# bonjour-l/esa-pose-estimation

Hardware: AMD Instinct MI355X
Metric: HRNet-W32 256x256 crops/sec (heatmaps + fused argmax/refine keypoints) (higher is better)
Workload: dtype bf16x6 (fp32-grade: every f32 operand split exactly into 3 bf16 terms, 6 bf16 MFMAs per product, f32 accumulate; f32 NHWC activations; f32 VALU stem conv1 / output layer) — heat-maps closer to fp64 than the fp32 CPU reference; 1 GPU; seg_hrnet2 HRNet-W32 256x256, batch 32/GPU, 11 keypoints, fp32 NCHW in -> heatmaps -> keypoints (BASELINE configs[1]); global_batch=32, per_gpu_batch=32, parallelism=dp1, hip_graph=True

## Files before the change

esa-pose-estimation_amd/csrc/conv_x6.hip:

```cpp
#include <algorithm>
#include <atomic>
#include <cstdio>
#include <type_traits>

#include "conv_cfg.h"
#include "devstate.h"
#include "kernels.h"
#include "sb.h"

#ifdef X6_TRACE
__device__ unsigned long long g_x6_trace[64 * 32 * 8];
extern "C" int esa_debug_x6_trace(void* dst) { return (int)hipMemcpyFromSymbol(dst, HIP_SYMBOL(g_x6_trace), sizeof(g_x6_trace)); }
__device__ unsigned long long g_x6_wg[1024 * 8];
extern "C" int esa_debug_x6_wg(void* dst) { return (int)hipMemcpyFromSymbol(dst, HIP_SYMBOL(g_x6_wg), sizeof(g_x6_wg)); }
#endif

#ifndef X6_ABL
#define X6_ABL 0
#endif
#ifndef X6_KG_SKEW
#define X6_KG_SKEW 1
#endif
#ifndef X6_W2BUF
#define X6_W2BUF 1
// ... 175 lines not shown
    auto advance = [&](const X6Pos& a) {
        X6Pos q = a;
        if (q.c + 1 < nchunks) {
            ++q.c;
        } else {
            q.c = 0;
            q.item += G;
            q.ok = a.ok && q.item < geo.nitems;
            if (q.ok) decode(q);
        }
        return q;
    };

    float* const w1s = reinterpret_cast<float*>(smem + C::LDS);
    constexpr int RW = C::IW + 2, RH = C::IH + 2, RAWN = RW * RH, RIT = STEM ? (RAWN + C::NT - 1) / C::NT : 1;
    float* const rawt = w1s + 2 * 4 * 10 * 8;
    if (STEM) {
        for (int i = tid; i < 2 * 4 * 10 * 8; i += C::NT) w1s[i] = stem.w1[i];
    }
    const int sg = tid & 3, q0 = tid >> 2;
    int qyx[XITER];
#pragma unroll
    for (int it = 0; it < XITER; ++it) {
        const int q = q0 + it * QSTEP;
        const int qy = q / C::IW, qx = q - qy * C::IW;
        qyx[it] = q < C::NPIX ? (qy << 8 | qx) : -1;
    }
    int roff[STEM ? XITER : 1];
    if constexpr (STEM) {
#pragma unroll
        for (int it = 0; it < XITER; ++it) roff[it] = qyx[it] >= 0 ? (qyx[it] >> 8) * RW + (qyx[it] & 255) : 0;
    }
    constexpr bool DEEP = !STEM && NBUF == 2 && (S == 2 || KS == 1) && X6_DEEP;
    constexpr int XH = (KS == 1 || DEEP || NBUF == 1) ? XITER : (XITER + 1) / 2;
    u32x4 xr[STEM ? 1 : XH][2];
// ... 66 lines not shown
                const int i = tid + k * C::NT;
                const int ry = i / RW, rx_ = i - ry * RW;
                const int yy = gy0 + ry, xx = gx0 + rx_;
                const bool in = i < RAWN && (unsigned)yy < (unsigned)p.H && (unsigned)xx < (unsigned)p.W;
                rawreg[k] = __builtin_bit_cast(float, __builtin_amdgcn_raw_buffer_load_b32(rx, in ? (yy * p.W + xx) * 4 : (int)X6_OOB, 0, 0));
            }
        }
    };
    auto raw_commit = [&](int rb) __attribute__((always_inline)) {
        if constexpr (STEM) {
#pragma unroll
            for (int k = 0; k < RIT; ++k)
                if (RAWN % C::NT == 0 || k + 1 < RIT || tid + k * C::NT < RAWN) rawt[rb * RAWN + tid + k * C::NT] = rawreg[k];
        }
    };
    auto stage_stem = [&](int buf, const X6Pos& q, int rb) __attribute__((always_inline)) {
        if constexpr (STEM) {
            const float* wt = w1s + (q.c * 4 + sg) * 80;
            const float* rt = rawt + rb * RAWN;
            const int gy0 = q.oy0 * S - C::PAD, gx0 = q.ox0 * S - C::PAD;
            constexpr int UG = XITER <= 3 ? 3 : 2;
            x6_static_for<0, (XITER + UG - 1) / UG>([&](auto g_c) __attribute__((always_inline)) {
                constexpr int u0 = decltype(g_c)::value * UG, un = XITER - u0 < UG ? XITER - u0 : UG;
                f32x4 a0[un], a1[un];
                {
                    const f32x4 b0 = *reinterpret_cast<const f32x4*>(wt + 72), b1 = *reinterpret_cast<const f32x4*>(wt + 76);
#pragma unroll
                    for (int u = 0; u < un; ++u) { a0[u] = b0; a1[u] = b1; }
                }
                x6_static_for<0, 9>([&](auto t_c) __attribute__((always_inline)) {
                    constexpr int t = decltype(t_c)::value;
                    const f32x4 w0 = *reinterpret_cast<const f32x4*>(wt + t * 8), w1v = *reinterpret_cast<const f32x4*>(wt + t * 8 + 4);
                    x6_static_for<0, un>([&](auto u_c) __attribute__((always_inline)) {
                        constexpr int u = decltype(u_c)::value;
                        const float v = rt[roff[u0 + u] + (t / 3) * RW + t % 3];
                        a0[u] = __builtin_elementwise_fma(f32x4{v, v, v, v}, w0, a0[u]);
                        a1[u] = __builtin_elementwise_fma(f32x4{v, v, v, v}, w1v, a1[u]);
                    });
                });
                x6_static_for<0, un>([&](auto u_c) __attribute__((always_inline)) {
                    constexpr int u = decltype(u_c)::value, it = u0 + u;
                    const int gy = gy0 + (qyx[it] >> 8), gx = gx0 + (qyx[it] & 255);
                    const uint32_t m = (qyx[it] >= 0 && (unsigned)gy < (unsigned)p.H && (unsigned)gx < (unsigned)p.W) ? 0xffffffffu : 0u;
                    u32x4 src[2];
#pragma unroll
                    for (int k = 0; k < 4; ++k) {
                        src[0][k] = __float_as_uint(relu1(a0[u][k])) & m;
                        src[1][k] = __float_as_uint(relu1(a1[u][k])) & m;
                    }
                    emit_unit(buf, it, src);
                });
                __builtin_amdgcn_sched_barrier(0);
// ... 694 lines not shown
    if (nblk <= 0 || nblk > 0x7fffffffLL) return (int)hipErrorInvalidValue;
    const int ntile16 = p.Coutp >> 4;
    long long want = (4LL * device_cus() + nblk - 1) / nblk;
    if (want > ntile16 / 4) want = ntile16 / 4;
    const int slices = want < 1 ? 1 : (int)want;
    const int per = (ntile16 + slices - 1) / slices;
    auto kern = conv1x1_x6_kernel<NCH, PG>;
    if (const int e_ = ensure_dyn_lds(reinterpret_cast<const void*>(kern), lds + per * 64)) return e_;
    hipLaunchKernelGGL(kern, dim3((unsigned)nblk, (unsigned)((ntile16 + per - 1) / per)), dim3(NTHREADS), lds + per * 64, stream, p, ntiles, tiles_per_row, per);
    return (int)hipGetLastError();
}

bool stem_fused_x6_supported(int cin, int cmid, int coutp) { return X6_MODE == 2 && cin == 1 && cmid == 64 && coutp % 64 == 0; }

void pack_stem_w1_x6(const float* w, const float* b, float* dst) {
    for (int c = 0; c < 2; ++c)
        for (int sg = 0; sg < 4; ++sg)
            for (int j = 0; j < 8; ++j) {
                const int ch = c * 32 + x6_chan_of_k(sg, j);
                float* o = dst + (c * 4 + sg) * 80;
                for (int t = 0; t < 9; ++t) o[t * 8 + j] = w[ch * 9 + t];
                o[72 + j] = b[ch];
            }
}

int launch_stem_fused_x6(const StemFusedParams& sp, hipStream_t stream) {
    if (!stem_fused_x6_supported(sp.cin, sp.Cmid, sp.Coutp)) return (int)hipErrorInvalidValue;
    using C = X6Cfg<3, 2, 4, X6_STEM_NR, 4, X6_STEM_NBUF>;
    ConvParams p{};
    p.x = nullptr; p.y = sp.y; p.res = nullptr; p.w = sp.w2; p.bias = sp.bias2;
    p.N = sp.N; p.H = sp.H; p.W = sp.W; p.OH = sp.OH; p.OW = sp.OW; p.Cinp = sp.Cmid; p.Coutp = sp.Coutp; p.relu = 1; p.fmt = FMT_F32;
    if (sp.OH != (sp.H + 1) / 2 || sp.OW != (sp.W + 1) / 2 || (long long)sp.H * sp.W * 4 >= 0x7fffffffLL ||
        (long long)sp.OH * sp.OW * sp.Coutp * 4 >= 0x7fffffffLL)
        return (int)hipErrorInvalidValue;
    X6Geo geo;
    geo.tiles_x = (p.OW + TW - 1) / TW;
    geo.tiles_y = (p.OH + C::TH - 1) / C::TH;
    geo.ctiles = p.Coutp / 64;
    const long long nitems = (long long)p.N * geo.tiles_y * geo.tiles_x * geo.ctiles;
    if (nitems <= 0 || nitems > 0x7fffffffLL) return (int)hipErrorInvalidValue;
    geo.nitems = (int)nitems;
    geo.m_ct = x6_magic(geo.ctiles);
    geo.m_tx = x6_magic(geo.tiles_x);
    geo.m_ty = x6_magic(geo.tiles_y);
    const int slots = 2 * device_cus();
    int grid = (int)(nitems < slots ? nitems : slots);
    if (grid > geo.ctiles) grid -= grid % geo.ctiles;
    constexpr int LDS = C::LDS + 2 * 4 * 10 * 8 * 4 + 2 * (C::IW + 2) * (C::IH + 2) * 4;
    if (const int e_ = ensure_dyn_lds(reinterpret_cast<const void*>(stem_x6_kernel), LDS)) return e_;
    X6StemSrc src{sp.x, sp.w1};
    hipLaunchKernelGGL(stem_x6_kernel, dim3((unsigned)grid), dim3(NTHREADS), LDS, stream, p, geo, src);
    return (int)hipGetLastError();
}

bool conv1x1_x6_supported(const ConvParams& p) {
    const int n = p.Cinp / 32;
    return p.fmt == FMT_F32 && !p.res && !p.out_f32 && p.nheads <= 1 && (p.Cinp % 32) == 0 && (p.Coutp % 16) == 0 && p.H == p.OH &&
           p.W == p.OW && (n == 1 || n == 2 || n == 3 || n == 4 || n == 6 || n == 8) && p.Coutp >= X6_C1_MINCOUT;
}
int launch_conv1x1_x6(const ConvParams& p, hipStream_t stream) {
    if (!conv1x1_x6_supported(p)) return (int)hipErrorInvalidValue;
    switch (p.Cinp / 32) {
        case 1: return launch_c1_x6_t<1, 2>(p, stream);
// ... 75 lines not shown
```

esa-pose-estimation_amd/csrc/head.hip:

```cpp
#include "devstate.h"
#include "gaussfit.h"
#include "kernels.h"
#include "refine.h"
#include "sb.h"

namespace esa {
namespace {

constexpr int FTW = 32;
constexpr int FIW = FTW + 2;
constexpr int FROW = FIW + 1;

struct LerpT {
    int i0, i1;
    float l0, l1;
};
__device__ __forceinline__ LerpT lerp_ac_true(int dst, int in, int out) {
    const float scale = out > 1 ? (float)(in - 1) / (float)(out - 1) : 0.f;
    const float src = scale * (float)dst;
    LerpT r;
    r.i0 = min((int)src, in - 1);
    r.i1 = r.i0 + (r.i0 < in - 1 ? 1 : 0);
    r.l1 = src - (float)r.i0;
    r.l0 = 1.f - r.l1;
// ... 35 lines not shown
        ld(r0 + lx.i1, v01);
        ld(r1 + lx.i0, v10);
        ld(r1 + lx.i1, v11);
#pragma unroll
        for (int i = 0; i < 8; ++i)
            v[i] = ly.l0 * (lx.l0 * v00[i] + lx.l1 * v01[i]) + ly.l1 * (lx.l0 * v10[i] + lx.l1 * v11[i]);
    }
}
__device__ __forceinline__ float final_stage_raw(const FinalParams& p, int n, int ci, int gy, int gx) {
    float v = 0.f;
    if (gy >= 0 && gy < p.H && gx >= 0 && gx < p.W)
        v = p.x0[(((size_t)n * p.cin + ci) * p.H + gy) * p.W + gx];
    return v;
}

template <int RPT>
__device__ __forceinline__ void final_tile_max(const FinalParams& p, const float* red, int tiles_x, int tiles_y) {
    constexpr int NP = FTW * 8 * RPT;
    const int lane = threadIdx.x & 63;
    const int ntiles = tiles_x * tiles_y, tile = (int)(blockIdx.x % (unsigned)ntiles), n = (int)(blockIdx.x / (unsigned)ntiles);
    const int oy0 = tile / tiles_x * (8 * RPT), ox0 = tile % tiles_x * FTW;
    for (int k = threadIdx.x >> 6; k < p.K; k += 4) {
        float bv = -INFINITY;
        int bi = 0x7fffffff;
#pragma unroll
        for (int j = 0; j < NP / 64; ++j) {
            const int q = lane + 64 * j, oy = oy0 + q / FTW, ox = ox0 + q % FTW;
            if (oy < p.H && ox < p.W) argmax_take(red[k * NP + q], oy * p.W + ox, bv, bi);
        }
#pragma unroll
// ... 6 lines not shown
    }
}

template <int KT, int RPT, bool KP>
__global__ __launch_bounds__(256) void final_kernel(FinalParams p, int tiles_x, int tiles_y) {
    constexpr int FTH = 8 * RPT, FIH = FTH + 2;
    extern __shared__ __attribute__((aligned(16))) char smem[];
    float* tile = reinterpret_cast<float*>(smem);
    const int CT = p.K + p.cin;
    int b = blockIdx.x;
    const int tx = b % tiles_x; b /= tiles_x;
    const int ty = b % tiles_y;
    const int n = b / tiles_y;
    const int oy0 = ty * FTH, ox0 = tx * FTW;

    constexpr int G = (KT + 7) >> 3;
    const float sc_y = final_scale(p.h, p.H), sc_x = final_scale(p.wd, p.W);
    for (int u = threadIdx.x; u < FIH * FIW * G; u += 256) {
        const int c8 = u % G;
        const int q = u / G;
        const int py = q / FIW, px = q - py * FIW;
        const int gy = oy0 - 1 + py, gx = ox0 - 1 + px;
        float v[8];
        final_stage8(p, n, gy, gx, c8, sc_y, sc_x, v);
#pragma unroll
        for (int i = 0; i < 8; ++i) {
            const int c = c8 * 8 + i;
            if (c < p.K) tile[(c * FIH + py) * FROW + px] = v[i];
        }
    }
    for (int u = threadIdx.x; u < FIH * FIW * p.cin; u += 256) {
        const int px = u % FIW;
        const int r = u / FIW;
        const int py = r % FIH, ci = r / FIH;
        tile[((p.K + ci) * FIH + py) * FROW + px] = final_stage_raw(p, n, ci, oy0 - 1 + py, ox0 - 1 + px);
    }
    __syncthreads();

    const int lx = threadIdx.x & (FTW - 1), lyy = (threadIdx.x / FTW) * RPT;
    if constexpr (RPT == 2) {
        f32x2 acc[KT];
#pragma unroll
        for (int k = 0; k < KT; ++k) acc[k] = f32x2{p.bias[k], p.bias[k]};
        for (int c = 0; c < CT; ++c) {
            const float* tp = tile + (c * FIH + lyy) * FROW + lx;
            const float* wp = p.w + (size_t)c * 9 * KT;
            float r[4][3];
#pragma unroll
            for (int i = 0; i < 4; ++i)
#pragma unroll
                for (int j = 0; j < 3; ++j) r[i][j] = tp[i * FROW + j];
// ... 66 lines not shown
    const int tiles_x = (p.W + FTW - 1) / FTW, tiles_y = (p.H + FTH - 1) / FTH;
    const long long nblk = (long long)p.N * tiles_x * tiles_y;
    if (nblk <= 0 || nblk > 0x7fffffffLL) return (int)hipErrorInvalidValue;
    const size_t lds = (size_t)(p.K + p.cin) * FIH * FROW * sizeof(float);
    auto kern = final_kernel<KT, RPT, KP>;
    if (const int e_ = ensure_dyn_lds(reinterpret_cast<const void*>(kern), 64 * 1024)) return e_;
    if (lds > 64 * 1024) return (int)hipErrorInvalidValue;
    hipLaunchKernelGGL(kern, dim3((unsigned)nblk), dim3(256), lds, stream, p, tiles_x, tiles_y);
    return (int)hipGetLastError();
}
inline int final_rpt(int K, int cin, int KT) { return (size_t)(K + cin) * 18 * FROW * sizeof(float) <= 64 * 1024 && KT <= 16 ? 2 : 1; }
template <int KT, bool KP = false>
int launch_final_t(const FinalParams& p, hipStream_t stream) {
    if (final_rpt(p.K, p.cin, KT) == 2) return launch_final_rt<KT, 2, KP>(p, stream);
    return launch_final_rt<KT, 1, KP>(p, stream);
}

constexpr int FKP_MAXC = 40;
__global__ __launch_bounds__(64) void final_kp_finish_kernel(FinalParams p, int kt, int ntiles, float* kp, int* idx_out) {
    __shared__ float sv[81][FKP_MAXC];
    __shared__ float spt[9];
    const int plane = blockIdx.x, n = plane / p.K, k = plane - n * p.K;
    float bv;
    int bi;
    reduce_tile_maxima(p.part + (size_t)plane * ntiles, ntiles, bv, bi);
    const int b0 = bi == 0x7fffffff ? 0 : bi, px = b0 % p.W, py = b0 / p.W;
    const int npt = 1 < px && px < p.W - 2 && 1 < py && py < p.H - 2 ? 9 : 1;
    const int G = (p.K + 7) >> 3, U = G + p.cin, CT = p.K + p.cin;
    const float sc_y = final_scale(p.h, p.H), sc_x = final_scale(p.wd, p.W);
    for (int u = threadIdx.x; u < npt * 9 * U; u += 64) {
// ... 492 lines not shown
            for (int l = 0; l < 64; ++l)
                for (int j = 0; j < 8; ++j) {
                    const int co = m * 16 + (l & 15), G = c * 4 + (l >> 4);
                    float v = 0.f;
                    if (G < 9 * cg_n) {
                        const int tap = G / cg_n, ch = (G % cg_n) * 8 + j;
                        if (co < K && ch < ct) v = w[((size_t)co * ct + ch) * 9 + tap];
                    }
                    const uint16_t hi = fb16(v), lo = fb16(v - fb16f(hi));
                    const size_t base = (((size_t)m * nch + c) * 2) * 512;
                    d[base + l * 8 + j] = hi;
                    d[base + 512 + l * 8 + j] = lo;
                }
}

int final_kp_tiles(int K, int cin, int H, int W) {
    const int kt = final_kt(K);
    if (kt < 0 || H <= 0 || W <= 0) return 0;
    return ((W + FTW - 1) / FTW) * ((H + 8 * final_rpt(K, cin, kt) - 1) / (8 * final_rpt(K, cin, kt)));
}

int launch_final_kp(const FinalParams& p, float* kp, int* idx_out, hipStream_t stream) {
    const int ntiles = final_kp_tiles(p.K, p.cin, p.H, p.W), kt = final_kt(p.K);
    const long long planes = (long long)p.N * p.K;
    if (!p.part || !kp || ntiles <= 0 || p.K + p.cin > FKP_MAXC || planes > 0x7fffffffLL || (long long)p.H * p.W > 0x7fffffffLL)
        return (int)hipErrorInvalidValue;
    int rc = (int)hipErrorInvalidValue;
    switch (kt) {
        case 11: rc = launch_final_t<11, true>(p, stream); break;
        case 16: rc = launch_final_t<16, true>(p, stream); break;
// ... 68 lines not shown
                case 31: return launch_final_mfma_t<3, 1, true>(p, stream);
                case 32: return launch_final_mfma_t<3, 2, true>(p, stream);
                case 42: return launch_final_mfma_t<4, 2, true>(p, stream);
                case 52: return launch_final_mfma_t<5, 2, true>(p, stream);
            }
        }
        switch (cg * 10 + m) {
            case 21: return launch_final_mfma_t<2, 1>(p, stream);
            case 31: return launch_final_mfma_t<3, 1>(p, stream);
            case 32: return launch_final_mfma_t<3, 2>(p, stream);
            case 42: return launch_final_mfma_t<4, 2>(p, stream);
            case 52: return launch_final_mfma_t<5, 2>(p, stream);
        }
    }
    if (p.fmt == FMT_HF) return (int)hipErrorInvalidValue;
    switch (final_kt(p.K)) {
        case 11: return launch_final_t<11>(p, stream);
        case 16: return launch_final_t<16>(p, stream);
        case 32: return launch_final_t<32>(p, stream);
    }
    return (int)hipErrorInvalidValue;
}

}
```

esa-pose-estimation_amd/csrc/kernels.h:

```cpp
#pragma once
#include <hip/hip_runtime.h>
#include <stdint.h>

namespace esa {

enum { FMT_SB = 0, FMT_BF = 1, FMT_F32 = 2, FMT_HF = 3 };
inline bool fmt_half(int fmt) { return fmt == FMT_BF || fmt == FMT_HF; }

int set_error(const char* fmt, ...);

struct ConvParams {
    const char* x;
    char* y;
    const char* res;
    const uint4* w;
    const float* bias;
    int N, H, W, OH, OW;
    int Cinp, Coutp;
    int relu;
    int out_f32;
    int fmt;
    int nheads;
    int x6_reload;
    char* yh[3];
// ... 58 lines not shown
    const float* bias2;
    int N, H, W;
};
int launch_bblock32(const BlockParams& p, hipStream_t stream);

struct StemFusedParams {
    const float* x;
    char* y;
    const float* w1;
    const float* bias1;
    const uint4* w2;
    const float* bias2;
    int N, H, W, OH, OW, cin, Cmid, Coutp;
};
int launch_stem_fused(const StemFusedParams& p, hipStream_t stream);
bool stem_fused_x6_supported(int cin, int cmid, int coutp);
void pack_stem_w1_x6(const float* w, const float* b, float* dst);
int launch_stem_fused_x6(const StemFusedParams& p, hipStream_t stream);

struct FuseParams {
    const char* x[4];
    int h[4], w[4];
    int nterms;
    char* y;
    int N, H, W, Cp;
    int relu;
    int fmt;
};
int launch_fuse(const FuseParams& p, hipStream_t stream);

struct FinalParams {
    const char* h3;
    const float* x0;
    float* out;
    const float* w;
    const float* bias;
    const uint4* wpk;
    int N, H, W, h, wd;
    int K, cin, Cp;
    int fmt;
    float2* part;
};
int launch_final(const FinalParams& p, hipStream_t stream);
int final_kp_tiles(int K, int cin, int H, int W);
int launch_final_kp(const FinalParams& p, float* kp, int* idx_out, hipStream_t stream);
int launch_final_gf(const FinalParams& p, float* kp, int* idx_out, double* fit, int* status, double* hess, hipStream_t stream);
int launch_final_gf_cov(const FinalParams& p, float* kp, int* idx_out, double* fit, int* status, double* hess, double* cov,
                        double* info, double cov_floor, hipStream_t stream);
int final2_valu_tiles(int H, int W);
int launch_final2_kp(const FinalParams& p, float* bmax, float* kp, int* idx_out, hipStream_t stream, double* hess = nullptr);
int final_part_tiles(int K, int cin, int H, int W);
__device__ __forceinline__ void argmax_take(float v, int i, float& bv, int& bi) {
    const bool vn = v != v, bn = bv != bv;
    if (v > bv || (vn && !bn) || ((v == bv || (vn && bn)) && i < bi)) { bv = v; bi = i; }
}
bool final_mfma_supported(int K, int cin);
size_t final_mfma_bytes(int K, int cin);
void pack_final_mfma(const float* w, int K, int cin, void* dst);

struct HeadParams {
    const char* x0;
    const char* t[3];
    char* y;
    const uint4* w0;
    const uint4* w3;
    const float* bias0;
    const float* bias3;
    int N, H, W;
    int th[3], tw[3];
    int C0p, Ctp, C3p, K;
    bool valu;
    bool hf;
};
// ... 194 lines not shown
```

esa-pose-estimation_amd/csrc/op_abi.hip:

```cpp
#include <algorithm>
#include <cstdint>
#include <cstdio>
#include <cstring>
#include <vector>

#include "../../include/esahrnet.h"
#include "host_util.h"
#include "kernels.h"

using esa::DevScope;
using esa::Format;
using esa::set_error;

static const float* f32(const void* p) { return static_cast<const float*>(p); }
static float* f32(void* p) { return static_cast<float*>(p); }
static bool aligned(const void* p, uintptr_t a) { return (reinterpret_cast<uintptr_t>(p) & (a - 1)) == 0; }

static bool conv_form_ok(int k, int stride) { return (k == 1 && stride == 1) || (k == 3 && (stride == 1 || stride == 2)); }
static bool op_conv_dims_ok(int n, int cin, int cout, int h, int w, int k, int stride) {
    if (n <= 0 || cin <= 0 || cout <= 0 || h <= 0 || w <= 0 || !conv_form_ok(k, stride)) return false;
    return (long long)n * h * w * (long long)((std::max(cin, cout) + 63) & ~63) * 4 <= 0x7fffffffLL;
}
static esa::ConvParams op_conv_shape(const Format& f, int n, int cin, int cout, int h, int w, int stride, int relu, const void* res) {
    esa::ConvParams p{};
// ... 305 lines not shown

int esahrnet_op_stem2(const void* x_dev, int n, int cin, int height, int width, const float* w1, const float* b1, int cmid,
                      const float* w2, const float* b2, int cout, int precision, void* y_dev, esahrnet_stream stream_) {
    const char* who = "op_stem2";
    if (!x_dev || !w1 || !b1 || !w2 || !b2 || !y_dev) return set_error("%s: null argument", who);
    if (precision != 0 && precision != 2) return set_error("%s: precision %d (0: stem_fused, 2: stem_x6_kernel)", who, precision);
    const Format f(precision);
    if (cin < 1 || cin > 4) return set_error("%s: cin=%d (1 .. 4)", who, cin);
    if (cmid <= 0 || (cmid & 31)) return set_error("%s: cmid=%d (a positive multiple of 32)", who, cmid);
    if (!op_conv_dims_ok(n, cmid, cout, height, width, 3, 2)) return set_error("%s: n=%d cmid=%d cout=%d %dx%d unsupported", who, n, cmid, cout, height, width);
    const int coutp = f.pad(cout), oh = (height + 1) / 2, ow = (width + 1) / 2;
    if (f.x6 && !esa::stem_fused_x6_supported(cin, cmid, coutp)) return set_error("%s: stem_x6_kernel does not serve cin=%d cmid=%d cout=%d", who, cin, cmid, cout);
    std::vector<float> w1p, b1p(b1, b1 + cmid), b2p(coutp, 0.f);
    std::copy(b2, b2 + cout, b2p.begin());
    if (f.x6) {
        w1p.assign(2 * 4 * 10 * 8, 0.f);
        esa::pack_stem_w1_x6(w1, b1, w1p.data());
    } else {
        w1p = esa::pack_stem_w(w1, cmid, cin, cmid);
    }
    DevScope m(who, static_cast<hipStream_t>(stream_));
    esa::StemFusedParams p{};
    p.x = f32(x_dev);
    p.N = n; p.H = height; p.W = width; p.OH = oh; p.OW = ow; p.cin = cin; p.Cmid = cmid; p.Coutp = coutp;
    if (m.upload(w1p, &p.w1) || m.upload(b1p, &p.bias1) || m.upload(f.pack(w2, cout, cmid, 3, coutp, cmid), &p.w2) || m.upload(b2p, &p.bias2)) return 1;
    if (m.alloc(&p.y, (size_t)n * oh * ow * coutp * 4)) return 1;
    int rc = f.x6 ? esa::launch_stem_fused_x6(p, m.stream()) : esa::launch_stem_fused(p, m.stream());
    if (!rc) rc = esa::launch_fmt_to_nchw(f.fmt, p.y, n, coutp, oh, ow, coutp, f32(y_dev), m.stream());
    return m.finish(rc);
}

// ... 69 lines not shown
```

esa-pose-estimation_amd/csrc/plan.hip:

```cpp
#include <hip/hip_runtime.h>

#include <algorithm>
#include <cmath>
#include <cstdarg>
#include <cstdio>
#include <cstdlib>
#include <cstring>
#include <map>
#include <string>
#include <vector>

#include "../../include/esahrnet.h"
#include "devstate.h"
#include "host_util.h"
#include "kernels.h"

namespace esa {
int final_kt(int K);
extern const int kFrontendMaxRows;
int check_boxes_args(const char* who, int m, int frame_h, int frame_w, int scale, int rule);
int check_crops_args(const char* who, int nframes, int pixel_format, float stdv);
int check_cov_args(const char* who, const void* cov_dev, const void* info_dev, double cov_floor);
int check_corr_args(const char* who, int m, int k, int mode);
}
// ... 107 lines not shown
};

enum StemForm { STEM_SEPARATE, STEM_FUSED, STEM_FUSED_X6 };
enum HeadForm { HEAD_UNFUSED, HEAD_SB, HEAD_BF, HEAD_X6 };

struct PlanOptions {
    bool unfused, head_v1, final_valu, no_multihead, no_jobs, no_bblock, no_cbam_jobs, cbam_unfused, stem_pool_separate,
         head3_direct, head3_cout32, bf_unfused_head, bf_head_valu, x6_unfused_head, x6_unfused_stem, x6_reload_weights, tap_all;
    int nlanes;
    int fmt;
    StemForm stem;
    bool fused_block;
    HeadForm head;
    bool head2;
    bool final_mfma;
};

PlanOptions plan_options(const esahrnet_cfg& g, const esa::Format& format) {
    const auto on = esa::env_on;
    PlanOptions o;
    o.unfused = on("ESAHRNET_UNFUSED"); o.head_v1 = on("ESAHRNET_HEAD_V1"); o.final_valu = on("ESAHRNET_FINAL_VALU");
    o.no_multihead = on("ESAHRNET_NO_MULTIHEAD"); o.no_jobs = on("ESAHRNET_NO_JOBS"); o.no_bblock = on("ESAHRNET_NO_BBLOCK");
    o.no_cbam_jobs = on("ESAHRNET_NO_CBAM_JOBS"); o.cbam_unfused = on("ESAHRNET_CBAM_UNFUSED");
    o.stem_pool_separate = on("ESAHRNET_STEM_POOL_SEPARATE"); o.head3_direct = on("ESAHRNET_HEAD3_DIRECT");
    o.head3_cout32 = on("ESAHRNET_HEAD3_COUT32"); o.bf_unfused_head = on("ESAHRNET_BF_UNFUSED_HEAD");
    o.bf_head_valu = on("ESAHRNET_BF_HEAD_VALU"); o.x6_unfused_head = on("ESAHRNET_X6_UNFUSED_HEAD");
    o.x6_unfused_stem = on("ESAHRNET_X6_UNFUSED_STEM"); o.tap_all = on("ESAHRNET_TAP_ALL");
    o.x6_reload_weights = on("ESAHRNET_X6_RELOAD_WEIGHTS");
    const char* streams = getenv("ESAHRNET_STREAMS");
    o.nlanes = streams && atoi(streams) > 1 ? 4 : 1;
// ... 1 lines not shown
    const bool sb = o.fmt == esa::FMT_SB, v0 = g.variant == 0;
    const bool x6_stem = esa::stem_fused_x6_supported(g.cin, pad32(g.stem_width), pad32(g.stem_width)) && g.stem_width == 64;
    o.stem = sb && (!v0 || !o.unfused) ? STEM_FUSED
           : o.fmt == esa::FMT_F32 && x6_stem && !o.x6_unfused_stem ? STEM_FUSED_X6 : STEM_SEPARATE;
    o.fused_block = sb && v0 && !o.unfused && !o.no_bblock;
    int nb4 = 0;
    while (nb4 < ESAHRNET_MAX_BRANCHES && g.blocks[3][nb4] > 0) ++nb4;
    const int c0 = pad32(g.widths[0]);
    o.head = !v0 || nb4 != 4 ? HEAD_UNFUSED
           : sb ? (!o.unfused && (c0 == 32 || c0 == 64) ? HEAD_SB : HEAD_UNFUSED)
           : esa::fmt_half(o.fmt) ? (!o.bf_unfused_head && (pad64(g.widths[0]) == 64 || pad64(g.widths[0]) == 128) ? HEAD_BF : HEAD_UNFUSED)
           : !o.x6_unfused_head && (c0 == 32 || c0 == 64) ? HEAD_X6 : HEAD_UNFUSED;
    o.head2 = !o.head_v1 && (o.head != HEAD_SB || ((pad32(g.widths[1]) == 64 || pad32(g.widths[1]) == 96) &&
                                                   esa::head_t_supported(pad32(g.widths[2])) && esa::head_t_supported(pad32(g.widths[3]))));
    o.final_mfma = v0 && o.fmt != esa::FMT_F32 && !o.final_valu && esa::final_mfma_supported(g.num_keypoints, g.cin);
    return o;
}

}

int esa::set_error(const char* fmt, ...) {
    va_list ap;
    va_start(ap, fmt);
    vsnprintf(g_err, sizeof g_err, fmt, ap);
    va_end(ap);
    return 1;
}

bool esa::conv_group_mergeable(int fmt, const esa::ConvParams* ps, int n, int k, int stride) {
    if (fmt == esa::FMT_F32) return esa::conv_x6_jobs_supported(ps, n, k, stride);
// ... 12 lines not shown
                  fmt == esa::FMT_HF ? "fp16" : esa::fmt_half(fmt) ? "true" : "false");
}

struct esahrnet_ctx {
    esahrnet_cfg cfg;
    int device;
    std::vector<ConvSpec> specs;
    std::map<std::string, int> spec_by_name;
    std::vector<DevConv> dconvs;
    std::vector<AuxSpec> aux;
    float *stemraw_w = nullptr, *stemraw_b = nullptr;
    std::vector<Tensor> tensors;
    std::vector<Op> ops;
    int spec_stem = -1, spec_final = -1;
    float *stem_w = nullptr, *stem_b = nullptr, *final_w = nullptr, *final_b = nullptr;
    void* final_wpk = nullptr;
    int spec_l0 = -1, spec_l3 = -1, head_c0 = 0;
    void *head_w0 = nullptr, *head_w3 = nullptr;
    float *head_b0 = nullptr, *head_b3 = nullptr;
    bool committed = false;
    bool keep = false;
    PlanOptions opt;
    esa::Format format;
    bool h16() const { return format.half; }
    bool hf() const { return format.hf; }
    bool x6() const { return format.x6; }
    int padc(int ch) const { return format.pad(ch); }
    int eb() const { return format.eb; }
    size_t wbytes(int coutp, int cinp, int k) const { return format.wbytes(coutp, cinp, k); }
    std::vector<char> pack(const float* w, int cout, int cin, int k, int coutp, int cinp) const { return format.pack(w, cout, cin, k, coutp, cinp); }
// ... 997 lines not shown
                if (allocated[ti] && last_of(t) == (int)oi) release(t.off, bytes_of(t));
            }
        high = std::max(high, top);
    }
    sp.bytes = high;
    c.sp = sp;
    return 0;
}

void free_weights(esahrnet_ctx& c) {
    for (DevConv& d : c.dconvs) {
        if (d.w) (void)hipFree(d.w);
        if (d.bias) (void)hipFree(d.bias);
        d.w = nullptr; d.bias = nullptr;
    }
    for (float** p : {&c.stem_w, &c.stem_b, &c.final_w, &c.final_b, &c.head_b0, &c.head_b3})
        if (*p) { (void)hipFree(*p); *p = nullptr; }
    for (void** p : {&c.head_w0, &c.head_w3, &c.final_wpk})
        if (*p) { (void)hipFree(*p); *p = nullptr; }
    for (AuxSpec& a : c.aux) if (a.dev) { (void)hipFree(a.dev); a.dev = nullptr; }
    for (Multi& m : c.multis) {
        if (m.w) (void)hipFree(m.w);
        if (m.bias) (void)hipFree(m.bias);
        m.w = nullptr; m.bias = nullptr;
    }
    for (float** p : {&c.stemraw_w, &c.stemraw_b}) if (*p) { (void)hipFree(*p); *p = nullptr; }
    for (std::vector<hipEvent_t>* v : {&c.wave_entry, &c.wave_end, &c.op_event}) {
        for (hipEvent_t& e : *v) if (e) { (void)hipEventDestroy(e); e = nullptr; }
        v->clear();
    }
    for (int i = 0; i < 3; ++i) {
// ... 259 lines not shown
        size_t wo = 0, bo = 0;
        for (int k = 0; k < m.n; ++k) {
            const DevConv& d = h->dconvs[h->ops[m.op[k]].dconv];
            const size_t wb = esa::packed_weight_bytes(d.coutp, d.cinp, 3);
            HIP_OK(hipMemcpy(static_cast<char*>(m.w) + wo, d.w, wb, hipMemcpyDeviceToDevice));
            HIP_OK(hipMemcpy(m.bias + bo, d.bias, (size_t)d.coutp * sizeof(float), hipMemcpyDeviceToDevice));
            wo += wb; bo += d.coutp;
        }
    }
    {
        const ConvSpec& s = h->specs[h->spec_stem];
        const int coutp = h->padc(s.cout);
        std::vector<float> w = pack_stem_w(s.w.data(), s.cout, s.cin, coutp), b(coutp, 0.f);
        std::copy(s.b.begin(), s.b.begin() + s.cout, b.begin());
        if (h->opt.stem == STEM_FUSED_X6) {
            std::vector<float> wx(2 * 4 * 10 * 8, 0.f);
            esa::pack_stem_w1_x6(s.w.data(), s.b.data(), wx.data());
            w = wx;
        }
        if (upload(w, reinterpret_cast<void**>(&h->stem_w)) || upload(b, reinterpret_cast<void**>(&h->stem_b))) return 1;
    }
    if (h->cfg.variant == 0) {
        const ConvSpec& s = h->specs[h->spec_final];
        const int kt = esa::final_kt(s.cout);
        std::vector<float> w((size_t)s.cin * 9 * kt, 0.f), b(std::max(kt, 32), 0.f);
        if (h->opt.final_mfma) {
            packed.assign(esa::final_mfma_bytes(s.cout, s.cin - s.cout), 0);
            esa::pack_final_mfma(s.w.data(), s.cout, s.cin - s.cout, packed.data());
            if (upload(packed, &h->final_wpk)) return 1;
        }
        for (int co = 0; co < s.cout; ++co) {
            b[co] = s.b[co];
            for (int ci = 0; ci < s.cin; ++ci)
                for (int t = 0; t < 9; ++t)
                    w[((size_t)ci * 9 + t) * kt + co] = s.w[((size_t)co * s.cin + ci) * 9 + t];
        }
        if (upload(w, reinterpret_cast<void**>(&h->final_w)) || upload(b, reinterpret_cast<void**>(&h->final_b))) return 1;
    }
    for (AuxSpec& a : h->aux)
        if (upload(a.data, reinterpret_cast<void**>(&a.dev))) return 1;
    for (const Op& o : h->ops)
        if (o.kind == OP_STEMRAW) {
            const AuxSpec& a = h->aux[o.aux[0]];
            const int cout = a.shape[0], cin = a.shape[1], coutp = h->padc(cout);
// ... 666 lines not shown
                p.x[i] = T(o.terms[i]); p.h[i] = lh[ti.level]; p.w[i] = lw[ti.level];
            }
            p.y = T(o.out); p.N = n; p.H = lh[to.level]; p.W = lw[to.level]; p.Cp = to.Cp;
            p.relu = o.relu; p.fmt = c.opt.fmt;
            if (desc) {
                describe(desc, c.hf() ? "fuse_kernel<fp16>" : "fuse_kernel", "fuse -> %s", to.tap.c_str());
                desc->bytes = tbytes(o.out);
                for (int i = 0; i < o.nterms; ++i) desc->bytes += tbytes(o.terms[i]);
            } else rc = esa::launch_fuse(p, stream);
            break;
        }
        case OP_FINAL: {
            const Tensor& ti = c.tensors[o.in];
            esa::FinalParams p{};
            p.h3 = T(o.in); p.x0 = static_cast<const float*>(b.x); p.out = static_cast<float*>(b.heat);
            p.w = c.final_w; p.bias = c.final_b; p.wpk = static_cast<const uint4*>(c.final_wpk);
            p.N = n; p.H = height; p.W = width; p.h = lh[ti.level]; p.wd = lw[ti.level];
            p.K = c.cfg.num_keypoints; p.cin = c.cfg.cin; p.Cp = ti.Cp; p.fmt = c.opt.fmt;
            p.part = static_cast<float2*>(b.part);
            if (desc) {
                const ConvSpec& s = c.specs[c.spec_final];
                describe(desc, c.hf() ? "final_kernel<fp16>" : "final_kernel", "%s", s.name.c_str());
                desc->flops = 2.0 * n * height * width * s.cout * s.cin * 9;
                desc->bytes = tbytes(o.in) + (double)n * height * width * (c.cfg.cin + s.cout) * 4;
            } else if (b.req.decoder != DEC_NONE)
                rc = run_decode(c, b, &p, nullptr, 0, 0, n, height, width, stream);
            else rc = esa::launch_final(p, stream);
            break;
        }
    }
    if (rc) return fail("forward: kernel launch failed: %s", hipGetErrorString((hipError_t)rc));
// ... 949 lines not shown
```

Measured before the change: 8116 crops/s.

## Move fp32 stem conv1 and final output conv onto f32 MFMA instructions

Replaces the VALU FMA loops in the fused stem's first 3x3 convolution with mfma_f32_16x16x4f32 instructions, repacking the stem weights into per-lane MFMA A-operand layout with the nine taps padded to twelve. It also adds a new f32 MFMA kernel for the final output conv, with packed weights plus per-step LDS tap offsets, selected when the format is fp32. The aim is to cut VALU time in the two full-resolution fp32 layers while keeping f32 accuracy. The cost is padded zero taps, extra weight packing and a new code path and layout to maintain.

```diff
diff --git a/esa-pose-estimation_amd/csrc/conv_x6.hip b/esa-pose-estimation_amd/csrc/conv_x6.hip
--- a/esa-pose-estimation_amd/csrc/conv_x6.hip
+++ b/esa-pose-estimation_amd/csrc/conv_x6.hip
@@ -213,11 +213,12 @@
 
     float* const w1s = reinterpret_cast<float*>(smem + C::LDS);
     constexpr int RW = C::IW + 2, RH = C::IH + 2, RAWN = RW * RH, RIT = STEM ? (RAWN + C::NT - 1) / C::NT : 1;
-    float* const rawt = w1s + 2 * 4 * 10 * 8;
+    float* const rawt = w1s + X6_STEM_W1;
     if (STEM) {
-        for (int i = tid; i < 2 * 4 * 10 * 8; i += C::NT) w1s[i] = stem.w1[i];
-    }
-    const int sg = tid & 3, q0 = tid >> 2;
+        for (int i = tid; i < X6_STEM_W1; i += C::NT) w1s[i] = stem.w1[i];
+    }
+    static_assert(!STEM || C::NT == 256, "the fused stem's staging map: four waves x 16 pixels per unit");
+    const int sg = STEM ? g : (tid & 3), q0 = STEM ? wave * 16 + px : (tid >> 2);
     int qyx[XITER];
 #pragma unroll
     for (int it = 0; it < XITER; ++it) {
@@ -314,28 +315,39 @@
                 if (RAWN % C::NT == 0 || k + 1 < RIT || tid + k * C::NT < RAWN) rawt[rb * RAWN + tid + k * C::NT] = rawreg[k];
         }
     };
+    int toff[STEM ? 3 : 1];
+    if constexpr (STEM) {
+#pragma unroll
+        for (int s = 0; s < 3; ++s) {
+            const int tap = 4 * s + g >= 3 ? 4 * s + g - 3 : 0;
+            toff[s] = (tap / 3) * RW + tap % 3;
+        }
+    }
     auto stage_stem = [&](int buf, const X6Pos& q, int rb) __attribute__((always_inline)) {
         if constexpr (STEM) {
-            const float* wt = w1s + (q.c * 4 + sg) * 80;
+            const float* wt = w1s + q.c * X6_STEM_W1_CHUNK;
             const float* rt = rawt + rb * RAWN;
             const int gy0 = q.oy0 * S - C::PAD, gx0 = q.ox0 * S - C::PAD;
-            constexpr int UG = XITER <= 3 ? 3 : 2;
+            float af[2][3];
+#pragma unroll
+            for (int mt = 0; mt < 2; ++mt)
+#pragma unroll
+                for (int s = 0; s < 3; ++s) af[mt][s] = wt[(mt * 3 + s) * 64 + lane];
+            const f32x4 b0 = *reinterpret_cast<const f32x4*>(wt + 384 + 4 * g), b1 = *reinterpret_cast<const f32x4*>(wt + 400 + 4 * g);
+            constexpr int UG = 3;
             x6_static_for<0, (XITER + UG - 1) / UG>([&](auto g_c) __attribute__((always_inline)) {
                 constexpr int u0 = decltype(g_c)::value * UG, un = XITER - u0 < UG ? XITER - u0 : UG;
                 f32x4 a0[un], a1[un];
-                {
-                    const f32x4 b0 = *reinterpret_cast<const f32x4*>(wt + 72), b1 = *reinterpret_cast<const f32x4*>(wt + 76);
-#pragma unroll
-                    for (int u = 0; u < un; ++u) { a0[u] = b0; a1[u] = b1; }
-                }
-                x6_static_for<0, 9>([&](auto t_c) __attribute__((always_inline)) {
-                    constexpr int t = decltype(t_c)::value;
-                    const f32x4 w0 = *reinterpret_cast<const f32x4*>(wt + t * 8), w1v = *reinterpret_cast<const f32x4*>(wt + t * 8 + 4);
+#pragma unroll
+                for (int u = 0; u < un; ++u) { a0[u] = b0; a1[u] = b1; }
+                x6_static_for<0, 3>([&](auto s_c) __attribute__((always_inline)) {
+                    constexpr int s = decltype(s_c)::value;
                     x6_static_for<0, un>([&](auto u_c) __attribute__((always_inline)) {
                         constexpr int u = decltype(u_c)::value;
-                        const float v = rt[roff[u0 + u] + (t / 3) * RW + t % 3];
-                        a0[u] = __builtin_elementwise_fma(f32x4{v, v, v, v}, w0, a0[u]);
-                        a1[u] = __builtin_elementwise_fma(f32x4{v, v, v, v}, w1v, a1[u]);
+                        float v = rt[roff[u0 + u] + toff[s]];
+                        if (s == 0) v = g == 3 ? v : 0.f;
+                        a0[u] = __builtin_amdgcn_mfma_f32_16x16x4f32(af[0][s], v, a0[u], 0, 0, 0);
+                        a1[u] = __builtin_amdgcn_mfma_f32_16x16x4f32(af[1][s], v, a1[u], 0, 0, 0);
                     });
                 });
                 x6_static_for<0, un>([&](auto u_c) __attribute__((always_inline)) {
@@ -1060,14 +1072,16 @@
 bool stem_fused_x6_supported(int cin, int cmid, int coutp) { return X6_MODE == 2 && cin == 1 && cmid == 64 && coutp % 64 == 0; }
 
 void pack_stem_w1_x6(const float* w, const float* b, float* dst) {
-    for (int c = 0; c < 2; ++c)
-        for (int sg = 0; sg < 4; ++sg)
-            for (int j = 0; j < 8; ++j) {
-                const int ch = c * 32 + x6_chan_of_k(sg, j);
-                float* o = dst + (c * 4 + sg) * 80;
-                for (int t = 0; t < 9; ++t) o[t * 8 + j] = w[ch * 9 + t];
-                o[72 + j] = b[ch];
-            }
+    for (int c = 0; c < 2; ++c) {
+        float* o = dst + c * X6_STEM_W1_CHUNK;
+        for (int mt = 0; mt < 2; ++mt)
+            for (int s = 0; s < 3; ++s)
+                for (int l = 0; l < 64; ++l) {
+                    const int ch = c * 32 + mt * 16 + (l & 15), k = 4 * s + (l >> 4);
+                    o[(mt * 3 + s) * 64 + l] = k < 3 ? 0.f : w[ch * 9 + (k - 3)];
+                }
+        for (int i = 0; i < 32; ++i) o[384 + i] = b[c * 32 + i];
+    }
 }
 
 int launch_stem_fused_x6(const StemFusedParams& sp, hipStream_t stream) {
@@ -1092,7 +1106,7 @@
     const int slots = 2 * device_cus();
     int grid = (int)(nitems < slots ? nitems : slots);
     if (grid > geo.ctiles) grid -= grid % geo.ctiles;
-    constexpr int LDS = C::LDS + 2 * 4 * 10 * 8 * 4 + 2 * (C::IW + 2) * (C::IH + 2) * 4;
+    constexpr int LDS = C::LDS + X6_STEM_W1 * 4 + 2 * (C::IW + 2) * (C::IH + 2) * 4;
     if (const int e_ = ensure_dyn_lds(reinterpret_cast<const void*>(stem_x6_kernel), LDS)) return e_;
     X6StemSrc src{sp.x, sp.w1};
     hipLaunchKernelGGL(stem_x6_kernel, dim3((unsigned)grid), dim3(NTHREADS), LDS, stream, p, geo, src);
diff --git a/esa-pose-estimation_amd/csrc/head.hip b/esa-pose-estimation_amd/csrc/head.hip
--- a/esa-pose-estimation_amd/csrc/head.hip
+++ b/esa-pose-estimation_amd/csrc/head.hip
@@ -73,6 +73,30 @@
     return v;
 }
 
+template <int G, int FIH>
+__device__ __forceinline__ void final_stage_tile(const FinalParams& p, float* tile, int n, int oy0, int ox0) {
+    const float sc_y = final_scale(p.h, p.H), sc_x = final_scale(p.wd, p.W);
+    for (int u = threadIdx.x; u < FIH * FIW * G; u += 256) {
+        const int c8 = u % G;
+        const int q = u / G;
+        const int py = q / FIW, px = q - py * FIW;
+        const int gy = oy0 - 1 + py, gx = ox0 - 1 + px;
+        float v[8];
+        final_stage8(p, n, gy, gx, c8, sc_y, sc_x, v);
+#pragma unroll
+        for (int i = 0; i < 8; ++i) {
+            const int c = c8 * 8 + i;
+            if (c < p.K) tile[(c * FIH + py) * FROW + px] = v[i];
+        }
+    }
+    for (int u = threadIdx.x; u < FIH * FIW * p.cin; u += 256) {
+        const int px = u % FIW;
+        const int r = u / FIW;
+        const int py = r % FIH, ci = r / FIH;
+        tile[((p.K + ci) * FIH + py) * FROW + px] = final_stage_raw(p, n, ci, oy0 - 1 + py, ox0 - 1 + px);
+    }
+}
+
 template <int RPT>
 __device__ __forceinline__ void final_tile_max(const FinalParams& p, const float* red, int tiles_x, int tiles_y) {
     constexpr int NP = FTW * 8 * RPT;
@@ -109,27 +133,7 @@
     const int n = b / tiles_y;
     const int oy0 = ty * FTH, ox0 = tx * FTW;
 
-    constexpr int G = (KT + 7) >> 3;
-    const float sc_y = final_scale(p.h, p.H), sc_x = final_scale(p.wd, p.W);
-    for (int u = threadIdx.x; u < FIH * FIW * G; u += 256) {
-        const int c8 = u % G;
-        const int q = u / G;
-        const int py = q / FIW, px = q - py * FIW;
-        const int gy = oy0 - 1 + py, gx = ox0 - 1 + px;
-        float v[8];
-        final_stage8(p, n, gy, gx, c8, sc_y, sc_x, v);
-#pragma unroll
-        for (int i = 0; i < 8; ++i) {
-            const int c = c8 * 8 + i;
-            if (c < p.K) tile[(c * FIH + py) * FROW + px] = v[i];
-        }
-    }
-    for (int u = threadIdx.x; u < FIH * FIW * p.cin; u += 256) {
-        const int px = u % FIW;
-        const int r = u / FIW;
-        const int py = r % FIH, ci = r / FIH;
-        tile[((p.K + ci) * FIH + py) * FROW + px] = final_stage_raw(p, n, ci, oy0 - 1 + py, ox0 - 1 + px);
-    }
+    final_stage_tile<(KT + 7) / 8, FIH>(p, tile, n, oy0, ox0);
     __syncthreads();
 
     const int lx = threadIdx.x & (FTW - 1), lyy = (threadIdx.x / FTW) * RPT;
@@ -226,6 +230,102 @@
 int launch_final_t(const FinalParams& p, hipStream_t stream) {
     if (final_rpt(p.K, p.cin, KT) == 2) return launch_final_rt<KT, 2, KP>(p, stream);
     return launch_final_rt<KT, 1, KP>(p, stream);
+}
+
+template <int NS, int RPT>
+__global__ __launch_bounds__(256) void final_f32mfma_kernel(FinalParams p, int tiles_x, int tiles_y, int ns, int pad) {
+    constexpr int FTH = 8 * RPT, FIH = FTH + 2, NR = 2 * RPT;
+    extern __shared__ __attribute__((aligned(16))) char smem[];
+    float* tile = reinterpret_cast<float*>(smem);
+    int b = blockIdx.x;
+    const int tx = b % tiles_x; b /= tiles_x;
+    const int ty = b % tiles_y;
+    const int n = b / tiles_y;
+    const int oy0 = ty * FTH, ox0 = tx * FTW;
+    const int lane = threadIdx.x & 63, wave = threadIdx.x >> 6, px = lane & 15, kq = lane >> 4;
+    const float* const wa = p.wf + lane;
+    const int* const wo = reinterpret_cast<const int*>(p.wf + (size_t)ns * 64) + kq;
+
+    float af[NS ? NS : 1];
+    int off[NS ? NS : 1];
+#pragma unroll
+    for (int s = 0; s < NS; ++s) { af[s] = wa[s * 64]; off[s] = wo[s * 4]; }
+
+    final_stage_tile<2, FIH>(p, tile, n, oy0, ox0);
+    __syncthreads();
+
+    f32x4 acc[NR][2];
+    {
+        const f32x4 bq = *reinterpret_cast<const f32x4*>(p.bias + 4 * kq);
+#pragma unroll
+        for (int r = 0; r < NR; ++r) { acc[r][0] = bq; acc[r][1] = bq; }
+    }
+    const float* const tb = tile + (wave * NR) * FROW + px;
+    auto step = [&](float a, int o, bool first) __attribute__((always_inline)) {
+        const float* t = tb + o;
+#pragma unroll
+        for (int r = 0; r < NR; ++r)
+#pragma unroll
+            for (int h = 0; h < 2; ++h) {
+                float v = t[r * FROW + 16 * h];
+                if (first) v = kq < pad ? 0.f : v;
+                acc[r][h] = __builtin_amdgcn_mfma_f32_16x16x4f32(a, v, acc[r][h], 0, 0, 0);
+            }
+    };
+    if constexpr (NS > 0) {
+#pragma unroll
+        for (int s = 0; s < NS; ++s) step(af[s], off[s], s == 0);
+    } else {
+        float a = wa[0];
+        int o = wo[0];
+        for (int s = 0; s < ns; ++s) {
+            const int s1 = s + 1 < ns ? s + 1 : s;
+            const float a1 = wa[s1 * 64];
+            const int o1 = wo[s1 * 4];
+            step(a, o, s == 0);
+            a = a1; o = o1;
+        }
+    }
+#pragma unroll
+    for (int r = 0; r < NR; ++r) {
+        const int oy = oy0 + wave * NR + r;
+#pragma unroll
+        for (int h = 0; h < 2; ++h) {
+            const int ox = ox0 + 16 * h + px;
+            if (oy < p.H && ox < p.W) {
+#pragma unroll
+                for (int j = 0; j < 4; ++j) {
+                    const int k = 4 * kq + j;
+                    if (k < p.K) p.out[(((size_t)n * p.K + k) * p.H + oy) * p.W + ox] = acc[r][h][j];
+                }
+            }
+        }
+    }
+}
+inline int final_f32mfma_pad(int K, int cin) { return (4 - (K + cin) * 9 % 4) % 4; }
+template <int NS, int RPT>
+int launch_final_f32mfma_t(const FinalParams& p, hipStream_t stream) {
+    constexpr int FTH = 8 * RPT, FIH = FTH + 2;
+    const int tiles_x = (p.W + FTW - 1) / FTW, tiles_y = (p.H + FTH - 1) / FTH;
+    const long long nblk = (long long)p.N * tiles_x * tiles_y;
+    if (nblk <= 0 || nblk > 0x7fffffffLL) return (int)hipErrorInvalidValue;
+    const size_t lds = (size_t)(p.K + p.cin) * FIH * FROW * sizeof(float);
+    if (lds > 64 * 1024) return (int)hipErrorInvalidValue;
+    const int pad = final_f32mfma_pad(p.K, p.cin), ns = ((p.K + p.cin) * 9 + pad) / 4;
+    auto kern = final_f32mfma_kernel<NS, RPT>;
+    if (const int e_ = ensure_dyn_lds(reinterpret_cast<const void*>(kern), 64 * 1024)) return e_;
+    hipLaunchKernelGGL(kern, dim3((unsigned)nblk), dim3(256), lds, stream, p, tiles_x, tiles_y, ns, pad);
+    return (int)hipGetLastError();
+}
+int launch_final_f32mfma(const FinalParams& p, hipStream_t stream) {
+    const int ns = ((p.K + p.cin) * 9 + 3) / 4;
+    if (final_rpt(p.K, p.cin, 16) == 1) return launch_final_f32mfma_t<0, 1>(p, stream);
+    switch (ns) {
+        case 14: return launch_final_f32mfma_t<14, 2>(p, stream);
+        case 27: return launch_final_f32mfma_t<27, 2>(p, stream);
+        case 39: return launch_final_f32mfma_t<39, 2>(p, stream);
+    }
+    return launch_final_f32mfma_t<0, 2>(p, stream);
 }
 
 constexpr int FKP_MAXC = 40;
@@ -748,6 +848,24 @@
                 }
 }
 
+int final_f32mfma_steps(int K, int cin) {
+    if (K < 1 || K > 16 || cin < 0) return 0;
+    if ((size_t)(K + cin) * 10 * FROW * sizeof(float) > 64 * 1024) return 0;
+    return ((K + cin) * 9 + 3) / 4;
+}
+size_t final_f32mfma_floats(int K, int cin) { return (size_t)final_f32mfma_steps(K, cin) * 68; }
+void pack_final_f32mfma(const float* w, int K, int cin, float* dst) {
+    const int ct = K + cin, pad = final_f32mfma_pad(K, cin), ns = final_f32mfma_steps(K, cin);
+    const int fih = 8 * final_rpt(K, cin, final_kt(K)) + 2;
+    int32_t* offs = reinterpret_cast<int32_t*>(dst + (size_t)ns * 64);
+    for (int s = 0; s < ns; ++s)
+        for (int l = 0; l < 64; ++l) {
+            const int m = l & 15, idx = 4 * s + (l >> 4) - pad;
+            dst[s * 64 + l] = idx >= 0 && m < K ? w[((size_t)m * ct + idx / 9) * 9 + idx % 9] : 0.f;
+            if (m == 0) offs[s * 4 + (l >> 4)] = idx >= 0 ? (idx / 9 * fih + idx % 9 / 3) * FROW + idx % 3 : 0;
+        }
+}
+
 int final_kp_tiles(int K, int cin, int H, int W) {
     const int kt = final_kt(K);
     if (kt < 0 || H <= 0 || W <= 0) return 0;
@@ -846,6 +964,7 @@
         }
     }
     if (p.fmt == FMT_HF) return (int)hipErrorInvalidValue;
+    if (p.fmt == FMT_F32 && p.wf && final_f32mfma_steps(p.K, p.cin)) return launch_final_f32mfma(p, stream);
     switch (final_kt(p.K)) {
         case 11: return launch_final_t<11>(p, stream);
         case 16: return launch_final_t<16>(p, stream);
diff --git a/esa-pose-estimation_amd/csrc/kernels.h b/esa-pose-estimation_amd/csrc/kernels.h
--- a/esa-pose-estimation_amd/csrc/kernels.h
+++ b/esa-pose-estimation_amd/csrc/kernels.h
@@ -96,6 +96,8 @@
     int N, H, W, OH, OW, cin, Cmid, Coutp;
 };
 int launch_stem_fused(const StemFusedParams& p, hipStream_t stream);
+constexpr int X6_STEM_W1_CHUNK = 2 * 3 * 64 + 32;
+constexpr int X6_STEM_W1 = 2 * X6_STEM_W1_CHUNK;
 bool stem_fused_x6_supported(int cin, int cmid, int coutp);
 void pack_stem_w1_x6(const float* w, const float* b, float* dst);
 int launch_stem_fused_x6(const StemFusedParams& p, hipStream_t stream);
@@ -118,6 +120,7 @@
     const float* w;
     const float* bias;
     const uint4* wpk;
+    const float* wf;
     int N, H, W, h, wd;
     int K, cin, Cp;
     int fmt;
@@ -139,6 +142,9 @@
 bool final_mfma_supported(int K, int cin);
 size_t final_mfma_bytes(int K, int cin);
 void pack_final_mfma(const float* w, int K, int cin, void* dst);
+int final_f32mfma_steps(int K, int cin);
+size_t final_f32mfma_floats(int K, int cin);
+void pack_final_f32mfma(const float* w, int K, int cin, float* dst);
 
 struct HeadParams {
     const char* x0;
diff --git a/esa-pose-estimation_amd/csrc/op_abi.hip b/esa-pose-estimation_amd/csrc/op_abi.hip
--- a/esa-pose-estimation_amd/csrc/op_abi.hip
+++ b/esa-pose-estimation_amd/csrc/op_abi.hip
@@ -343,7 +343,7 @@
     std::vector<float> w1p, b1p(b1, b1 + cmid), b2p(coutp, 0.f);
     std::copy(b2, b2 + cout, b2p.begin());
     if (f.x6) {
-        w1p.assign(2 * 4 * 10 * 8, 0.f);
+        w1p.assign(esa::X6_STEM_W1, 0.f);
         esa::pack_stem_w1_x6(w1, b1, w1p.data());
     } else {
         w1p = esa::pack_stem_w(w1, cmid, cin, cmid);
diff --git a/esa-pose-estimation_amd/csrc/plan.hip b/esa-pose-estimation_amd/csrc/plan.hip
--- a/esa-pose-estimation_amd/csrc/plan.hip
+++ b/esa-pose-estimation_amd/csrc/plan.hip
@@ -145,6 +145,7 @@
     HeadForm head;
     bool head2;
     bool final_mfma;
+    bool final_f32mfma;
 };
 
 PlanOptions plan_options(const esahrnet_cfg& g, const esa::Format& format) {
@@ -176,6 +177,7 @@
     o.head2 = !o.head_v1 && (o.head != HEAD_SB || ((pad32(g.widths[1]) == 64 || pad32(g.widths[1]) == 96) &&
                                                    esa::head_t_supported(pad32(g.widths[2])) && esa::head_t_supported(pad32(g.widths[3]))));
     o.final_mfma = v0 && o.fmt != esa::FMT_F32 && !o.final_valu && esa::final_mfma_supported(g.num_keypoints, g.cin);
+    o.final_f32mfma = v0 && o.fmt == esa::FMT_F32 && !o.final_valu && esa::final_f32mfma_steps(g.num_keypoints, g.cin) > 0;
     return o;
 }
 
@@ -218,6 +220,7 @@
     std::vector<Op> ops;
     int spec_stem = -1, spec_final = -1;
     float *stem_w = nullptr, *stem_b = nullptr, *final_w = nullptr, *final_b = nullptr;
+    float* final_wf = nullptr;
     void* final_wpk = nullptr;
     int spec_l0 = -1, spec_l3 = -1, head_c0 = 0;
     void *head_w0 = nullptr, *head_w3 = nullptr;
@@ -1245,7 +1248,7 @@
         if (d.bias) (void)hipFree(d.bias);
         d.w = nullptr; d.bias = nullptr;
     }
-    for (float** p : {&c.stem_w, &c.stem_b, &c.final_w, &c.final_b, &c.head_b0, &c.head_b3})
+    for (float** p : {&c.stem_w, &c.stem_b, &c.final_w, &c.final_wf, &c.final_b, &c.head_b0, &c.head_b3})
         if (*p) { (void)hipFree(*p); *p = nullptr; }
     for (void** p : {&c.head_w0, &c.head_w3, &c.final_wpk})
         if (*p) { (void)hipFree(*p); *p = nullptr; }
@@ -1535,7 +1538,7 @@
         std::vector<float> w = pack_stem_w(s.w.data(), s.cout, s.cin, coutp), b(coutp, 0.f);
         std::copy(s.b.begin(), s.b.begin() + s.cout, b.begin());
         if (h->opt.stem == STEM_FUSED_X6) {
-            std::vector<float> wx(2 * 4 * 10 * 8, 0.f);
+            std::vector<float> wx(esa::X6_STEM_W1, 0.f);
             esa::pack_stem_w1_x6(s.w.data(), s.b.data(), wx.data());
             w = wx;
         }
@@ -1549,6 +1552,11 @@
             packed.assign(esa::final_mfma_bytes(s.cout, s.cin - s.cout), 0);
             esa::pack_final_mfma(s.w.data(), s.cout, s.cin - s.cout, packed.data());
             if (upload(packed, &h->final_wpk)) return 1;
+        }
+        if (h->opt.final_f32mfma) {
+            std::vector<float> wf(esa::final_f32mfma_floats(s.cout, s.cin - s.cout), 0.f);
+            esa::pack_final_f32mfma(s.w.data(), s.cout, s.cin - s.cout, wf.data());
+            if (upload(wf, reinterpret_cast<void**>(&h->final_wf))) return 1;
         }
         for (int co = 0; co < s.cout; ++co) {
             b[co] = s.b[co];
@@ -2245,7 +2253,7 @@
             const Tensor& ti = c.tensors[o.in];
             esa::FinalParams p{};
             p.h3 = T(o.in); p.x0 = static_cast<const float*>(b.x); p.out = static_cast<float*>(b.heat);
-            p.w = c.final_w; p.bias = c.final_b; p.wpk = static_cast<const uint4*>(c.final_wpk);
+            p.w = c.final_w; p.bias = c.final_b; p.wpk = static_cast<const uint4*>(c.final_wpk); p.wf = c.final_wf;
             p.N = n; p.H = height; p.W = width; p.h = lh[ti.level]; p.wd = lw[ti.level];
             p.K = c.cfg.num_keypoints; p.cin = c.cfg.cin; p.Cp = ti.Cp; p.fmt = c.opt.fmt;
             p.part = static_cast<float2*>(b.part);
```

After: 8015 crops/s. 0.988x the previous value.
